# zer0int/OpenVision

Hardware: AMD Instinct MI355X
Metric: images/sec (node) ViT-L/14@224 fwd+InfoNCE (higher is better)
Workload: dtype bf16; 1 GPU; vit-large-patch14-224: image tower + text tower (T=80) + InfoNCE, per-GPU batch 256, formula weights, bf16 MFMA / fp32 accumulate; fp8_mask=0, global_batch=256, micro_batches=1, parallelism=dp1

## Files before the change

include/ovhip.h:

```cpp
#ifndef OVHIP_H
#define OVHIP_H

#include <stddef.h>
#include <stdint.h>

#ifdef __cplusplus
extern "C" {
#endif

#define OV_ABI_VERSION 2

typedef void* ov_stream_t;
typedef uint16_t ov_bf16;

enum ov_status {
    OV_OK = 0,
    OV_ERR_INVALID = -1,
    OV_ERR_UNSUPPORTED = -2,
    OV_ERR_WORKSPACE = -3,
    OV_ERR_NO_DEVICE = -4,
    OV_ERR_HIP = -1000
};

enum ov_dtype { OV_F32 = 0, OV_BF16 = 1 };
// ... 29 lines not shown
int ov_gemm_ln(const ov_bf16* X, int64_t ldx, const ov_bf16* Wg, int64_t ldw, const float* cvec, const float* colsum,
               const float* rowstats, ov_bf16* C, int64_t ldc, int64_t M, int N, int K, int epilogue, ov_stream_t stream);

int ov_gemm_keep(const ov_bf16* A, int64_t lda, const ov_bf16* W, int64_t ldw, const float* bias, ov_bf16* C, int64_t ldc,
                 ov_bf16* C2, int64_t ldc2, int64_t M, int N, int K, int epilogue, ov_stream_t stream);

int ov_rowstats(const ov_bf16* x, int64_t ldx, float* rowstats, int64_t rows, int D, float eps, ov_stream_t stream);

int ov_rowparts(const ov_bf16* x, int64_t ldx, float* parts, int64_t rows, int D, ov_stream_t stream);
int ov_rowstats_finalize(const float* parts, float* rowstats, int64_t rows, int D, float eps, ov_stream_t stream);
int ov_gemm_rowparts(const ov_bf16* A, int64_t lda, const ov_bf16* W, int64_t ldw, const float* bias, ov_bf16* C, int64_t ldc,
                     int64_t M, int N, int K, const ov_bf16* R, int64_t ldr, float* parts, ov_stream_t stream);

int ov_attention(const ov_bf16* qkv, int64_t ld_qkv, ov_bf16* out, int64_t ld_out,
                 int B, int L, int H, int hd, float scale, ov_stream_t stream);
int ov_attention_lse(const ov_bf16* qkv, int64_t ld_qkv, ov_bf16* out, int64_t ld_out, float* lse, int B, int L, int H, int hd, float scale,
                     ov_stream_t stream);
int ov_attention_prefix(const ov_bf16* qkv, int64_t ld_qkv, ov_bf16* out, int64_t ld_out, int B, int L, int H, int hd, float scale,
                        int prefix, ov_stream_t stream);

int ov_im2col_patches(const void* image, int img_dtype, ov_bf16* out, int B, int S, int P, int Kpad,
                      ov_stream_t stream);

int ov_im2col_patches_keep(const void* image, int img_dtype, const int* keep, ov_bf16* out, int B, int S, int P, int K, int Kpad,
                           ov_stream_t stream);
int ov_patch_keep_inverse(const int* keep, int* inv, int B, int K, int G, int* err_flag, ov_stream_t stream);
int ov_patch_keep_assemble(const ov_bf16* y, int64_t ldy, const float* cls, const float* pos, const int* keep, float* x, int B, int K,
                           int G, int D, ov_stream_t stream);
int ov_patch_keep_assemble_backward(const float* dx, const int* inv, int B, int K, int G, int D, float* dpos, float* dcls, ov_bf16* dy,
                                    int64_t lddy, ov_stream_t stream);
// ... 153 lines not shown
ov_tower* ov_tower_create(const ov_tower_cfg* cfg);
void      ov_tower_destroy(ov_tower* t);
int       ov_tower_set_block(ov_tower* t, int layer, const ov_block_weights* w);
int       ov_tower_set_block_fp8(ov_tower* t, int layer, const ov_block_fp8* q);
int       ov_tower_set_fp8_hidden_scale(ov_tower* t, float* amax, int mode);
#define OV_FP8_QKV 1
#define OV_FP8_OUT 2
#define OV_FP8_FC 4
#define OV_FP8_PROJ 8
#define OV_FP8_ALL 15
int       ov_tower_set_fp8_mask(ov_tower* t, const unsigned char* mask, int n);
int       ov_tower_set_prefix(ov_tower* t, int prefix);
size_t    ov_tower_workspace_bytes(const ov_tower* t, int B, int L);
int       ov_tower_forward(const ov_tower* t, ov_bf16* x, int B, int L, void* workspace,
                           size_t workspace_bytes, ov_stream_t stream);

typedef struct {
    float *ln1_w, *ln1_b;
    ov_bf16* qkv_w; float* qkv_b;
    ov_bf16* out_w; float* out_b;
    float *ln2_w, *ln2_b;
    ov_bf16* fc_w;  float* fc_b;
    ov_bf16* proj_w; float* proj_b;
} ov_block_grads;
typedef struct {
    const ov_bf16* qkv;
    const ov_bf16* attn_out;
    const ov_bf16* x1;
    const ov_bf16* fc_pre;
    const ov_bf16* ln1_out;
// ... 104 lines not shown
```

openvision_amd/_lib.py:

```python
from __future__ import annotations

import ctypes as C
import os
import threading

_PKG = os.path.dirname(os.path.abspath(__file__))
LIB_PATH = os.path.join(_PKG, "libovhip.so")
if os.environ.get("OVHIP_LIB"):
    LIB_PATH = os.path.join(_PKG, os.environ["OVHIP_LIB"]) if os.sep not in os.environ["OVHIP_LIB"] else os.environ["OVHIP_LIB"]

OV_F32, OV_BF16 = 0, 1
EPI_BIAS, EPI_GELU_ERF, EPI_GELU_TANH, EPI_RESIDUAL = 0, 1, 2, 3

c_void_p, c_int, c_int64, c_float, c_size_t = C.c_void_p, C.c_int, C.c_int64, C.c_float, C.c_size_t


class TowerCfg(C.Structure):
    _fields_ = [("width", c_int), ("layers", c_int), ("heads", c_int), ("mlp", c_int), ("mlp_pad", c_int),
                ("gelu_tanh", c_int), ("ln_eps", c_float)]


class BlockWeights(C.Structure):
    _fields_ = [(n, c_void_p) for n in ("ln1_w", "ln1_b", "qkv_w", "qkv_b", "out_w", "out_b", "ln2_w", "ln2_b",
                                        "fc_w", "fc_b", "proj_w", "proj_b", "qkv_colsum", "fc_colsum")]
# ... 42 lines not shown
                                   c_void_p, c_int64, c_int, c_int, c_int, c_void_p, c_int64, c_void_p]),
    "ov_tower_set_fp8_hidden_scale": (c_int, [c_void_p, c_void_p, c_int]),
    "ov_tower_set_fp8_mask": (c_int, [c_void_p, c_void_p, c_int]),
    "ov_layernorm_quant_fp8": (c_int, [c_void_p, c_int64, c_void_p, c_void_p, c_void_p, c_int64, c_void_p, c_int64, c_int, c_float,
                                       c_void_p]),
    "ov_gemm_ln": (c_int, [c_void_p, c_int64, c_void_p, c_int64, c_void_p, c_void_p, c_void_p, c_void_p, c_int64, c_int64, c_int,
                           c_int, c_int, c_void_p]),
    "ov_gemm_keep": (c_int, [c_void_p, c_int64, c_void_p, c_int64, c_void_p, c_void_p, c_int64, c_void_p, c_int64, c_int64, c_int, c_int,
                             c_int, c_void_p]),
    "ov_rowstats": (c_int, [c_void_p, c_int64, c_void_p, c_int64, c_int, c_float, c_void_p]),
    "ov_rowparts": (c_int, [c_void_p, c_int64, c_void_p, c_int64, c_int, c_void_p]),
    "ov_rowstats_finalize": (c_int, [c_void_p, c_void_p, c_int64, c_int, c_float, c_void_p]),
    "ov_gemm_rowparts": (c_int, [c_void_p, c_int64, c_void_p, c_int64, c_void_p, c_void_p, c_int64, c_int64, c_int, c_int, c_void_p, c_int64,
                                 c_void_p, c_void_p]),
    "ov_attention": (c_int, [c_void_p, c_int64, c_void_p, c_int64, c_int, c_int, c_int, c_int, c_float, c_void_p]),
    "ov_attention_prefix": (c_int, [c_void_p, c_int64, c_void_p, c_int64, c_int, c_int, c_int, c_int, c_float, c_int, c_void_p]),
    "ov_attention_prefix_backward_workspace_bytes": (c_size_t, [c_int, c_int, c_int, c_int]),
    "ov_attention_prefix_backward": (c_int, [c_void_p, c_int64, c_void_p, c_int64, c_void_p, c_int64, c_void_p, c_int64, c_int, c_int, c_int,
                                             c_int, c_float, c_int, c_void_p, c_size_t, c_void_p]),
    "ov_softmax_xent_workspace_bytes": (c_size_t, [c_int64]),
    "ov_softmax_xent": (c_int, [c_void_p, c_int64, c_void_p, c_void_p, c_int64, c_int, c_void_p, c_void_p, c_void_p, c_size_t, c_void_p]),
    "ov_softmax_xent_backward": (c_int, [c_void_p, c_int64, c_void_p, c_void_p, c_void_p, c_void_p, c_void_p, c_int64, c_int64, c_int,
                                         c_void_p, c_size_t, c_void_p]),
    "ov_tower_set_prefix": (c_int, [c_void_p, c_int]),
    "ov_block_backward_prefix": (c_int, [c_void_p, c_void_p, c_void_p, c_void_p, c_void_p, c_void_p, c_void_p, c_int, c_int, c_int, c_void_p,
                                         c_size_t, c_void_p]),
    "ov_im2col_patches": (c_int, [c_void_p, c_int, c_void_p, c_int, c_int, c_int, c_int, c_void_p]),
    "ov_im2col_patches_keep": (c_int, [c_void_p, c_int, c_void_p, c_void_p, c_int, c_int, c_int, c_int, c_int, c_void_p]),
    "ov_patch_keep_inverse": (c_int, [c_void_p, c_void_p, c_int, c_int, c_int, c_void_p, c_void_p]),
    "ov_patch_keep_assemble": (c_int, [c_void_p, c_int64, c_void_p, c_void_p, c_void_p, c_void_p, c_int, c_int, c_int, c_int, c_void_p]),
# ... 73 lines not shown
                                      c_void_p, c_void_p, c_void_p, c_void_p, c_void_p, c_void_p, c_void_p, c_size_t, c_void_p]),
    "ov_adamw_step": (c_int, [c_void_p, c_void_p, c_void_p, c_void_p, c_int64, c_float, c_float, c_float, c_float, c_float, c_int, c_float,
                              c_void_p, c_float, c_void_p]),
    "ov_sumsq_workspace_bytes": (c_size_t, []),
    "ov_sumsq": (c_int, [c_void_p, c_int64, c_void_p, c_int, c_void_p, c_size_t, c_void_p]),
    "ov_profile_enable": (c_int, [C.c_uint, c_int]),
    "ov_profile_read": (c_int, [c_int, C.POINTER(C.c_double), C.POINTER(c_int), C.POINTER(C.c_double)]),
    "ov_debug_gemm_stamps": (c_int, [c_void_p, c_int]),
    "ov_debug_gemm_wave_stamps": (c_int, [c_void_p]),
    "ov_tower_create": (c_void_p, [C.POINTER(TowerCfg)]),
    "ov_tower_destroy": (None, [c_void_p]),
    "ov_tower_set_block": (c_int, [c_void_p, c_int, C.POINTER(BlockWeights)]),
    "ov_tower_set_block_fp8": (c_int, [c_void_p, c_int, c_void_p]),
    "ov_tower_workspace_bytes": (c_size_t, [c_void_p, c_int, c_int]),
    "ov_tower_forward": (c_int, [c_void_p, c_void_p, c_int, c_int, c_void_p, c_size_t, c_void_p]),
    "ov_vision_workspace_bytes": (c_size_t, [c_void_p, C.POINTER(VisionHead), c_int]),
    "ov_vision_embed": (c_int, [c_void_p, C.POINTER(VisionHead), c_void_p, c_int, c_int, c_void_p, c_void_p, c_size_t,
                                c_void_p]),
    "ov_vision_head_forward": (c_int, [c_void_p, C.POINTER(VisionHead), c_void_p, c_int, c_void_p, c_int, c_void_p,
                                       c_size_t, c_void_p]),
    "ov_encode_image": (c_int, [c_void_p, C.POINTER(VisionHead), c_void_p, c_int, c_int, c_void_p, c_int, c_void_p,
                                c_size_t, c_void_p]),
    "ov_vision_head_forward_tokens": (c_int, [c_void_p, C.POINTER(VisionHead), c_void_p, c_int, c_int, c_void_p, c_int, c_void_p,
                                              c_size_t, c_void_p]),
    "ov_vision_keep_workspace_bytes": (c_size_t, [c_void_p, C.POINTER(VisionHead), c_int, c_int]),
    "ov_vision_embed_keep": (c_int, [c_void_p, C.POINTER(VisionHead), c_void_p, c_int, c_void_p, c_int, c_int, c_void_p, c_void_p,
                                     c_void_p, c_size_t, c_void_p]),
    "ov_encode_image_keep": (c_int, [c_void_p, C.POINTER(VisionHead), c_void_p, c_int, c_void_p, c_int, c_int, c_void_p, c_int,
                                     c_void_p, c_void_p, c_size_t, c_void_p]),
    "ov_text_workspace_bytes": (c_size_t, [c_void_p, C.POINTER(TextHead), c_int]),
# ... 48 lines not shown
```

openvision_amd/csrc/attention.hip:

```cpp
#include "common.h"
#include <stdlib.h>

namespace {

struct AttnArgs {
    const ov_bf16* qkv; int64_t ldq;
    ov_bf16* out; int64_t ldo;
    int B, L, H, nqt, KC;
    float scale_log2;
    int prefix;
};

typedef __attribute__((address_space(3))) s16x4_t* lds_s16x4_ptr;
typedef const __attribute__((address_space(1))) void* gptr_t;
typedef __attribute__((address_space(3))) void* lptr_t;

__device__ __forceinline__ bf16x8_t tr_pair(const char* p0, const char* p1) {
    const s16x4_t a = __builtin_amdgcn_ds_read_tr16_b64_v4i16((lds_s16x4_ptr)p0);
    const s16x4_t b = __builtin_amdgcn_ds_read_tr16_b64_v4i16((lds_s16x4_ptr)p1);
    typedef short s16x8_t __attribute__((ext_vector_type(8)));
    const s16x8_t c = {a[0], a[1], a[2], a[3], b[0], b[1], b[2], b[3]};
    return __builtin_bit_cast(bf16x8_t, c);
}

// ... 810 lines not shown
    const float inv = 1.0f / l;
    const int q = q0 + r;
    if (q < L) {
        ov_bf16* op = a.out + ((int64_t)b * L + q) * a.ldo + h * hd + 4 * h2;
#pragma unroll
        for (int t = 0; t < DT; ++t)
#pragma unroll
            for (int g = 0; g < 4; ++g) {
                const int d = t * 32 + 8 * g + 4 * h2;
                if (d < hd) {
                    const u32x2_t w = {pack_bf16x2(o[t][4 * g] * inv, o[t][4 * g + 1] * inv),
                                       pack_bf16x2(o[t][4 * g + 2] * inv, o[t][4 * g + 3] * inv)};
                    *(u32x2_t*)(op + t * 32 + 8 * g) = w;
                }
            }
    }
}

}

namespace {
int attention_impl(const ov_bf16* qkv, int64_t ld_qkv, ov_bf16* out, int64_t ld_out, int B, int L, int H, int hd, float scale,
                   const float* out_amax, float* amax_next, float* lse, ov_stream_t stream);
}

extern "C" int ov_attention(const ov_bf16* qkv, int64_t ld_qkv, ov_bf16* out, int64_t ld_out, int B, int L,
                            int H, int hd, float scale, ov_stream_t stream) {
    return attention_impl(qkv, ld_qkv, out, ld_out, B, L, H, hd, scale, nullptr, nullptr, nullptr, stream);
}

// ... 144 lines not shown
    static OvPerDeviceOnce attr;
    const int dev = ov_current_device();
    if (attr.need(dev)) {
        hipError_t e = hipFuncSetAttribute((const void*)attn_fwd_generic<64, true>, hipFuncAttributeMaxDynamicSharedMemorySize, 160 * 1024);
        if (e == hipSuccess)
            e = hipFuncSetAttribute((const void*)attn_fwd_generic<96, true>, hipFuncAttributeMaxDynamicSharedMemorySize, 160 * 1024);
        if (e != hipSuccess) return OV_ERR_HIP - (int)e;
        attr.mark(dev);
    }
    const dim3 grid((unsigned)(B * H), (unsigned)((g.nqt + nwg - 1) / nwg)), blk(nwg * 64);
    if (hdp == 64) hipLaunchKernelGGL((attn_fwd_generic<64, true>), grid, blk, smem, (hipStream_t)stream, g, hd);
    else hipLaunchKernelGGL((attn_fwd_generic<96, true>), grid, blk, smem, (hipStream_t)stream, g, hd);
    OV_LAUNCH_CHECK();
    return OV_OK;
}
```

openvision_amd/csrc/tower.hip:

```cpp
#include "common.h"
#include <new>
#include <vector>
#include <mutex>
#include <stdlib.h>

struct TailCtx {
    hipStream_t stream = nullptr;
    hipEvent_t fork = nullptr, join = nullptr;
    int state = 0;
    int device = -1;
    std::mutex mu;
};

struct ov_tower {
    mutable TailCtx tail;
    ov_tower_cfg cfg;
    ov_block_weights* blocks;
    unsigned char* set;
    ov_block_fp8* fp8;
    unsigned char* set8;
    float* h_amax;
    int h_mode;
    unsigned char* mask8;
    int prefix;
// ... 34 lines not shown
        e0 = g_prof.pool.back(); g_prof.pool.pop_back();
        e1 = g_prof.pool.back(); g_prof.pool.pop_back();
        on = true;
        (void)hipEventRecord(e0, st);
    }
    ~ProfScope() {
        if (!on) return;
        (void)hipEventRecord(e1, st);
        std::lock_guard<std::mutex> lk(g_prof.mu);
        g_prof.recs.push_back({cls, e0, e1, rows});
    }
};

inline size_t align_up(size_t x, size_t a) { return (x + a - 1) / a * a; }
inline int max_i(int a, int b) { return a > b ? a : b; }

struct VisionWs { size_t x, tower, pooled, lnrow, feat, total; };
inline VisionWs vision_ws(const ov_tower* t, const ov_vision_head* h, int B) {
    const int g = h->image_size / h->patch_size, L = g * g + 1, D = t->cfg.width;
    VisionWs w;
    size_t off = 0;
    w.x = off;      off += align_up((size_t)B * L * D * 2, 256);
    w.tower = off;  off += align_up(ov_tower_workspace_bytes(t, B, L), 256);
    w.pooled = off; off += align_up((size_t)B * D * 4, 256);
    w.lnrow = off;  off += align_up((size_t)B * D * 2, 256);
    w.feat = off;   off += align_up((size_t)B * h->embed_pad * 2, 256);
    w.total = off;
    return w;
}
inline size_t keep_embed_bytes(const ov_tower* t, const ov_vision_head* h, int B, int K) {
// ... 187 lines not shown
    }
    return OV_OK;
}

extern "C" int ov_tower_set_prefix(ov_tower* t, int prefix) {
    if (!t || prefix < -1) return OV_ERR_INVALID;
    t->prefix = prefix;
    return OV_OK;
}

extern "C" size_t ov_tower_workspace_bytes(const ov_tower* t, int B, int L) {
    if (!t || B <= 0 || L <= 0) return 0;
    const size_t M = (size_t)B * L;
    const int D = t->cfg.width;
    size_t n = align_up(M * D * 2, 256) + align_up(M * (size_t)big_pitch(t->cfg) * 2, 256) + align_up(M * 8, 256) +
               align_up(M * (size_t)(D / 32) * 8, 256);
    if (tower_fp8(t)) n += align_up(M * (size_t)max_i(D, t->cfg.mlp_pad), 256) + align_up(M * 4, 256);
    return n;
}

namespace {
struct BlockPart { ov_bf16 *x, *h, *big; float *stats, *parts; unsigned char* q8; float* qs; int B; ov_stream_t stream; bool prof; };
struct Fp8Scales { float *h_amax, *a_amax, *h_next, *a_next; int h_mode; };

int run_block(const ov_tower_cfg& c, const ov_block_weights& w, const ov_block_fp8* q, int mask, const Fp8Scales& sc, const BlockPart& p,
              bool parts_in, int L, int prefix) {
    const int D = c.width, H = c.heads, hd = D / H, F = c.mlp_pad, B = p.B;
    const int64_t M = (int64_t)B * L;
    const int ldb = big_pitch(c);
    const float scale = 1.0f / sqrtf((float)hd);
// ... 59 lines not shown
        else if (fold) OV_STEP(fc_cls, ov_gemm_ln(x, D, w.fc_w, D, w.fc_b, w.fc_colsum, stats, big, ldb, M, F, D, gelu, stream));
        else OV_STEP(fc_cls, ov_gemm(h, D, w.fc_w, D, w.fc_b, big, ldb, M, F, D, gelu, nullptr, 0, 0, 0, 0, stream));
        if (f_proj) {
            OV_STEP(OV_PROF_LN, ov_quant_rows_fp8(big, ldb, q8, F, qs, M, F, (sc.h_mode == 1 && f_fc) ? sc.h_amax : nullptr, stream));
            OV_STEP(OV_PROF_GEMM_PROJ, ov_gemm_fp8(q8, F, q->proj_w8, F, qs, q->proj_s, w.proj_b, x, D, M, D, F, OV_EPI_BIAS_RESIDUAL, x, D, stream));
        } else if (rp) {
            OV_STEP(OV_PROF_GEMM_PROJ, ov_gemm_rowparts(big, ldb, w.proj_w, F, w.proj_b, x, D, M, D, F, x, D, parts, stream));
        } else {
            OV_STEP(OV_PROF_GEMM_PROJ, ov_gemm(big, ldb, w.proj_w, F, w.proj_b, x, D, M, D, F, OV_EPI_BIAS_RESIDUAL, x, D, 0, 0, 0, stream));
        }
    }
#undef OV_STEP
    return OV_OK;
}

TailCtx* tail_ctx(const ov_tower* t) {
    TailCtx& tc = t->tail;
    std::lock_guard<std::mutex> lk(tc.mu);
    if (tc.state == 0) {
        const char* e = getenv("OVHIP_NO_TAIL_SPLIT");
        if (e && e[0] == '1') { tc.state = -1; return nullptr; }
        tc.device = ov_current_device();
        if (hipStreamCreateWithFlags(&tc.stream, hipStreamNonBlocking) == hipSuccess &&
            hipEventCreateWithFlags(&tc.fork, hipEventDisableTiming) == hipSuccess &&
            hipEventCreateWithFlags(&tc.join, hipEventDisableTiming) == hipSuccess)
            tc.state = 1;
        else
            tc.state = -1;
    }
    return tc.state == 1 && tc.device == ov_current_device() ? &tc : nullptr;
}

int tail_images(int B, int L) {
    const int64_t T = ((int64_t)B * L + 255) / 256;
    const int r = (int)(T % 64);
    if (T <= 64 || r == 0 || r > 8) return 0;
    const int64_t target = T - r;
    int Bm = (int)((target * 256) / L);
    while (Bm > 0 && ((int64_t)Bm * L + 255) / 256 > target) --Bm;
    const int tail = B - Bm;
    if (Bm <= 0 || tail <= 0 || tail > B / 8) return 0;
    return tail;
}
}

extern "C" int ov_tower_forward(const ov_tower* t, ov_bf16* x, int B, int L, void* workspace, size_t workspace_bytes,
                                ov_stream_t stream) {
    if (!t || !x || !workspace || B <= 0 || L <= 0) return OV_ERR_INVALID;
    if (workspace_bytes < ov_tower_workspace_bytes(t, B, L)) return OV_ERR_WORKSPACE;
    if (((uintptr_t)x | (uintptr_t)workspace) & 15) return OV_ERR_INVALID;
    const ov_tower_cfg& c = t->cfg;
    const int D = c.width;
    const int64_t M = (int64_t)B * L;
    const int ldb = big_pitch(c);
    ov_bf16* h = (ov_bf16*)workspace;
    ov_bf16* big = (ov_bf16*)((char*)workspace + align_up((size_t)M * D * 2, 256));
    float* stats = (float*)((char*)big + align_up((size_t)M * ldb * 2, 256));
    for (int i = 0; i < c.layers; ++i)
        if (!t->set[i]) return OV_ERR_INVALID;

    int nt = tail_images(B, L);
    TailCtx* tc = nt > 0 ? tail_ctx(t) : nullptr;
    if (!tc) nt = 0;
    const int Bm = B - nt;
    hipStream_t main_st = (hipStream_t)stream;
// ... 7 lines not shown
    const int64_t off = (int64_t)Bm * L;
    const bool fp8 = tower_fp8(t);
    if (t->prefix >= 0 && fp8) return OV_ERR_UNSUPPORTED;
    if (t->prefix > L) return OV_ERR_INVALID;
    int rc = OV_OK;
    if (fp8 && t->h_amax && t->h_mode == 2)
        rc = ov_amax_roll(t->h_amax, t->h_amax + 2 * c.layers, 2 * c.layers, stream);
    const int G = D / 32;
    float* parts = use_rowparts() && !fp8 ? (float*)((char*)workspace + ov_tower_workspace_bytes(t, B, L) - align_up((size_t)M * G * 8, 256)) : nullptr;
    const int qw = D > c.mlp_pad ? D : c.mlp_pad;
    unsigned char* q8 = (unsigned char*)stats + align_up((size_t)M * 8, 256);
    float* qs = (float*)(q8 + align_up((size_t)M * qw, 256));
    const BlockPart main_part = {x, h, big, stats, parts, q8, qs, Bm, stream, true};
    const BlockPart tail_part = {x + off * D, h + off * D, big + off * ldb, stats + 2 * off, parts ? parts + 2 * off * G : nullptr,
                                 q8 + off * qw, qs + off, nt, (ov_stream_t)(nt > 0 ? tc->stream : nullptr), false};
    for (int i = 0; i < c.layers && rc == OV_OK; ++i) {
        Fp8Scales sc = {nullptr, nullptr, nullptr, nullptr, 0};
        if (t->h_amax) sc = {t->h_amax + i, t->h_amax + c.layers + i, t->h_amax + 2 * c.layers + i, t->h_amax + 3 * c.layers + i, t->h_mode};
        const ov_block_fp8* q = fp8 ? &t->fp8[i] : nullptr;
        const int mask = fp8 ? t->mask8[i] : 0;
        rc = run_block(c, t->blocks[i], q, mask, sc, main_part, i > 0, L, t->prefix);
        if (rc == OV_OK && nt > 0) rc = run_block(c, t->blocks[i], q, mask, sc, tail_part, i > 0, L, t->prefix);
    }
    if (nt > 0) {
        hipError_t e = hipEventRecord(tc->join, tc->stream);
        if (e == hipSuccess) e = hipStreamWaitEvent(main_st, tc->join, 0);
        if (e != hipSuccess && rc == OV_OK) rc = OV_ERR_HIP - (int)e;
    }
    return rc;
}

int block_grad_pairs(const ov_block_grads* g);
int block_backward_partial(const ov_tower_cfg* cfg, const ov_block_weights* w, const ov_bf16* x, const ov_block_saved* s, const ov_bf16* dy,
                           ov_bf16* dx, const ov_block_grads* g, int prefix, int B, int L, void* workspace, size_t workspace_bytes,
                           ov_stream_t stream);
size_t block_backward_input_workspace_bytes(const ov_tower_cfg* cfg, int B, int L);
int block_backward_input(const ov_tower_cfg* cfg, const ov_block_weights* w, const ov_bf16* x, const ov_block_saved* s, const ov_bf16* dy,
                         ov_bf16* dx, int prefix, int B, int L, void* workspace, ov_stream_t stream);

static inline size_t saved_per_token(const ov_tower_cfg& c) { return (size_t)8 * c.width + 2 * (size_t)c.mlp_pad; }
static inline size_t saved_lse_elems(const ov_tower_cfg& c, int B, int L) {
    return ((size_t)2 * B * c.heads * ((L + 31) / 32 * 32) + 7) / 8 * 8;
}
static inline size_t saved_per_layer(const ov_tower_cfg& c, int B, int L) { return (size_t)B * L * saved_per_token(c) + saved_lse_elems(c, B, L); }
// ... 255 lines not shown
    int rc;
    if ((rc = ov_im2col_patches(image, img_dtype, patches, B, h->image_size, h->patch_size, h->kpad, stream))) return rc;
    if ((rc = ov_gemm(patches, h->kpad, h->conv_w, h->kpad, nullptr, x, D, (int64_t)B * g * g, D, h->kpad,
                      OV_EPI_BIAS_RESIDUAL, h->pos, D, g * g, g * g, 1, stream)))
        return rc;
    return ov_cls_rows(x, D, h->cls, h->pos_f32, B, L, D, stream);
}

extern "C" int ov_vision_head_forward(const ov_tower* t, const ov_vision_head* h, const ov_bf16* x, int B, float* features,
                                      int normalize, void* workspace, size_t workspace_bytes, ov_stream_t stream) {
    if (!t || !h || !x || !features || !workspace || B <= 0 || h->patch_size <= 0) return OV_ERR_INVALID;
    const int g = h->image_size / h->patch_size;
    return ov_vision_head_forward_tokens(t, h, x, B, g * g + 1, features, normalize, workspace, workspace_bytes, stream);
}

extern "C" int ov_vision_head_forward_tokens(const ov_tower* t, const ov_vision_head* h, const ov_bf16* x, int B, int L, float* features,
                                             int normalize, void* workspace, size_t workspace_bytes, ov_stream_t stream) {
    if (!t || !h || !x || !features || !workspace || B <= 0 || L < 2) return OV_ERR_INVALID;
    const int D = t->cfg.width, E = h->embed_dim, EP = h->embed_pad;
    if (EP % 8 || EP < E) return OV_ERR_INVALID;
    if (!h->final_ln_after_pool) return OV_ERR_UNSUPPORTED;
    const size_t o_pooled = 0, o_ln = align_up((size_t)B * D * 4, 256), o_feat = o_ln + align_up((size_t)B * D * 2, 256);
    if (workspace_bytes < o_feat + (size_t)B * EP * 2) return OV_ERR_WORKSPACE;
    float* pooled = (float*)((char*)workspace + o_pooled);
    ov_bf16* ln = (ov_bf16*)((char*)workspace + o_ln);
    ov_bf16* feat = (ov_bf16*)((char*)workspace + o_feat);
    int rc;
    if (h->pool_avg) {
        if ((rc = ov_mean_pool(x, D, pooled, B, L, D, 1, stream))) return rc;
        if ((rc = ov_layernorm(pooled, OV_F32, D, h->ln_post_w, h->ln_post_b, ln, OV_BF16, D, B, D, t->cfg.ln_eps, stream))) return rc;
    } else {
        if ((rc = ov_layernorm(x, OV_BF16, (int64_t)L * D, h->ln_post_w, h->ln_post_b, ln, OV_BF16, D, B, D, t->cfg.ln_eps, stream)))
            return rc;
    }
    if ((rc = ov_gemm(ln, D, h->proj_t, D, nullptr, feat, EP, B, EP, D, OV_EPI_BIAS, nullptr, 0, 0, 0, 0, stream))) return rc;
    if (normalize) return ov_l2norm(feat, OV_BF16, EP, features, E, B, E, stream);
    return ov_convert(feat, OV_BF16, EP, features, OV_F32, E, B, E, stream);
}

extern "C" int ov_encode_image(const ov_tower* t, const ov_vision_head* h, const void* image, int img_dtype, int B,
                               float* features, int normalize, void* workspace, size_t workspace_bytes, ov_stream_t stream) {
    if (!t || !h || !image || !features || !workspace || B <= 0) return OV_ERR_INVALID;
    const VisionWs w = vision_ws(t, h, B);
    if (workspace_bytes < w.total) return OV_ERR_WORKSPACE;
    const int g = h->image_size / h->patch_size, L = g * g + 1;
    char* ws = (char*)workspace;
    ov_bf16* x = (ov_bf16*)(ws + w.x);
    const size_t tower_bytes = ov_tower_workspace_bytes(t, B, L);
    int rc;
    if ((size_t)B * g * g * h->kpad * 2 > tower_bytes) return OV_ERR_WORKSPACE;
    if ((rc = ov_vision_embed(t, h, image, img_dtype, B, x, ws + w.tower, tower_bytes, stream))) return rc;
    if ((rc = ov_tower_forward(t, x, B, L, ws + w.tower, tower_bytes, stream))) return rc;
    return ov_vision_head_forward(t, h, x, B, features, normalize, ws + w.pooled, w.total - w.pooled, stream);
}

int ov_im2col_patches_keep_pos(const void* image, int img_dtype, const int* keep, ov_bf16* out, int B, int S, int P, int K, int Kpad,
                               const ov_bf16* pos, ov_bf16* posk, int D, int* err_flag, ov_stream_t stream);

extern "C" size_t ov_vision_keep_workspace_bytes(const ov_tower* t, const ov_vision_head* h, int B, int K) {
    if (!t || !h || B <= 0 || h->patch_size <= 0) return 0;
    const int g = h->image_size / h->patch_size;
    if (K < 1 || K > g * g) return 0;
    return vision_keep_ws(t, h, B, K).total;
}

extern "C" int ov_vision_embed_keep(const ov_tower* t, const ov_vision_head* h, const void* image, int img_dtype, const int* keep, int B,
                                    int K, ov_bf16* x, int* err_flag, void* workspace, size_t workspace_bytes, ov_stream_t stream) {
    if (!t || !h || !image || !keep || !x || !workspace || B <= 0 || h->patch_size <= 0) return OV_ERR_INVALID;
// ... 14 lines not shown
}

extern "C" int ov_encode_image_keep(const ov_tower* t, const ov_vision_head* h, const void* image, int img_dtype, const int* keep, int B,
                                    int K, float* features, int normalize, int* err_flag, void* workspace, size_t workspace_bytes,
                                    ov_stream_t stream) {
    if (!t || !h || !image || !keep || !features || !workspace || B <= 0 || h->patch_size <= 0) return OV_ERR_INVALID;
    const int g = h->image_size / h->patch_size;
    if (K < 1 || K > g * g) return OV_ERR_INVALID;
    const VisionWs w = vision_keep_ws(t, h, B, K);
    if (workspace_bytes < w.total) return OV_ERR_WORKSPACE;
    const int L = K + 1;
    char* ws = (char*)workspace;
    ov_bf16* x = (ov_bf16*)(ws + w.x);
    int rc;
    if ((rc = ov_vision_embed_keep(t, h, image, img_dtype, keep, B, K, x, err_flag, ws + w.tower, w.pooled - w.tower, stream))) return rc;
    if ((rc = ov_tower_forward(t, x, B, L, ws + w.tower, w.pooled - w.tower, stream))) return rc;
    return ov_vision_head_forward_tokens(t, h, x, B, L, features, normalize, ws + w.pooled, w.total - w.pooled, stream);
}

extern "C" size_t ov_text_workspace_bytes(const ov_tower* t, const ov_text_head* h, int B) {
    if (!t || !h || B <= 0) return 0;
    return text_ws(t, h, B).total;
}

extern "C" int ov_encode_text(const ov_tower* t, const ov_text_head* h, const int64_t* tokens, int B, float* features,
                              int normalize, int* err_flag, void* workspace, size_t workspace_bytes, ov_stream_t stream) {
    if (!t || !h || !tokens || !features || !workspace || B <= 0) return OV_ERR_INVALID;
    const TextWs w = text_ws(t, h, B);
    if (workspace_bytes < w.total) return OV_ERR_WORKSPACE;
    const int T = h->context_length, D = t->cfg.width, E = h->embed_dim, EP = (E + 7) / 8 * 8;
    char* ws = (char*)workspace;
    ov_bf16* x = (ov_bf16*)(ws + w.x);
    ov_bf16* last = (ov_bf16*)(ws + w.last);
    ov_bf16* ln = (ov_bf16*)(ws + w.lnrow);
    ov_bf16* feat = (ov_bf16*)(ws + w.feat);
    int rc;
    if ((rc = ov_text_embed(tokens, h->token_embedding, h->pos, x, D, B, T, D, h->vocab_size, err_flag, stream))) return rc;
    if ((rc = ov_tower_forward(t, x, B, T, ws + w.tower, ov_tower_workspace_bytes(t, B, T), stream))) return rc;
    if ((rc = ov_gather_rows(x, D, last, D, B, T, h->pool_last ? T - 1 : 0, D, stream))) return rc;
    if ((rc = ov_layernorm(last, OV_BF16, D, h->ln_final_w, h->ln_final_b, ln, OV_BF16, D, B, D, t->cfg.ln_eps, stream))) return rc;
    if ((rc = ov_gemm(ln, D, h->proj_t, D, nullptr, feat, EP, B, EP, D, OV_EPI_BIAS, nullptr, 0, 0, 0, 0, stream))) return rc;
    if (normalize) return ov_l2norm(feat, OV_BF16, EP, features, E, B, E, stream);
    return ov_convert(feat, OV_BF16, EP, features, OV_F32, E, B, E, stream);
}
```

Before: 5690 images/sec.

## Compute only pooled token rows in final transformer block

The last transformer block now computes K/V for all tokens but runs Q projection, attention, output projection, LN2 and the MLP only for the pooled row (CLS for vision, last/first token for text). A new row-wise attention kernel handles single query rows against full K/V. This removes most of the final layer's GEMM and attention cost in both towers. It adds a separate code path with extra workspace and a scalar attention kernel, and falls back to the full path for fp8 or prefix modes.

Result: no change. 5716 images/sec, median of 6 (+0.5%).

```diff
diff --git a/include/ovhip.h b/include/ovhip.h
--- a/include/ovhip.h
+++ b/include/ovhip.h
@@ -67,6 +67,8 @@
 
 int ov_attention(const ov_bf16* qkv, int64_t ld_qkv, ov_bf16* out, int64_t ld_out,
                  int B, int L, int H, int hd, float scale, ov_stream_t stream);
+int ov_attention_rows(const ov_bf16* q, int64_t ldq, const ov_bf16* kv, int64_t ldkv, ov_bf16* out, int64_t ldo,
+                      int B, int L, int H, int hd, float scale, ov_stream_t stream);
 int ov_attention_lse(const ov_bf16* qkv, int64_t ld_qkv, ov_bf16* out, int64_t ld_out, float* lse, int B, int L, int H, int hd, float scale,
                      ov_stream_t stream);
 int ov_attention_prefix(const ov_bf16* qkv, int64_t ld_qkv, ov_bf16* out, int64_t ld_out, int B, int L, int H, int hd, float scale,
@@ -250,6 +252,8 @@
 size_t    ov_tower_workspace_bytes(const ov_tower* t, int B, int L);
 int       ov_tower_forward(const ov_tower* t, ov_bf16* x, int B, int L, void* workspace,
                            size_t workspace_bytes, ov_stream_t stream);
+int       ov_tower_forward_pooled(const ov_tower* t, ov_bf16* x, int B, int L, int row, ov_bf16* out_rows, void* workspace,
+                                  size_t workspace_bytes, ov_stream_t stream);
 
 typedef struct {
     float *ln1_w, *ln1_b;
diff --git a/openvision_amd/_lib.py b/openvision_amd/_lib.py
--- a/openvision_amd/_lib.py
+++ b/openvision_amd/_lib.py
@@ -80,6 +80,7 @@
     "ov_gemm_rowparts": (c_int, [c_void_p, c_int64, c_void_p, c_int64, c_void_p, c_void_p, c_int64, c_int64, c_int, c_int, c_void_p, c_int64,
                                  c_void_p, c_void_p]),
     "ov_attention": (c_int, [c_void_p, c_int64, c_void_p, c_int64, c_int, c_int, c_int, c_int, c_float, c_void_p]),
+    "ov_attention_rows": (c_int, [c_void_p, c_int64, c_void_p, c_int64, c_void_p, c_int64, c_int, c_int, c_int, c_int, c_float, c_void_p]),
     "ov_attention_prefix": (c_int, [c_void_p, c_int64, c_void_p, c_int64, c_int, c_int, c_int, c_int, c_float, c_int, c_void_p]),
     "ov_attention_prefix_backward_workspace_bytes": (c_size_t, [c_int, c_int, c_int, c_int]),
     "ov_attention_prefix_backward": (c_int, [c_void_p, c_int64, c_void_p, c_int64, c_void_p, c_int64, c_void_p, c_int64, c_int, c_int, c_int,
@@ -183,6 +184,7 @@
     "ov_tower_set_block_fp8": (c_int, [c_void_p, c_int, c_void_p]),
     "ov_tower_workspace_bytes": (c_size_t, [c_void_p, c_int, c_int]),
     "ov_tower_forward": (c_int, [c_void_p, c_void_p, c_int, c_int, c_void_p, c_size_t, c_void_p]),
+    "ov_tower_forward_pooled": (c_int, [c_void_p, c_void_p, c_int, c_int, c_int, c_void_p, c_void_p, c_size_t, c_void_p]),
     "ov_vision_workspace_bytes": (c_size_t, [c_void_p, C.POINTER(VisionHead), c_int]),
     "ov_vision_embed": (c_int, [c_void_p, C.POINTER(VisionHead), c_void_p, c_int, c_int, c_void_p, c_void_p, c_size_t,
                                 c_void_p]),
diff --git a/openvision_amd/csrc/attention.hip b/openvision_amd/csrc/attention.hip
--- a/openvision_amd/csrc/attention.hip
+++ b/openvision_amd/csrc/attention.hip
@@ -848,6 +848,107 @@
                     *(u32x2_t*)(op + t * 32 + 8 * g) = w;
                 }
             }
+    }
+}
+
+struct AttnRowArgs {
+    const ov_bf16* q; int64_t ldq;
+    const ov_bf16* kv; int64_t ldkv;
+    ov_bf16* out; int64_t ldo;
+    int L, H, hd;
+    float scale_log2;
+};
+constexpr int ROW_KEYS = 128;
+constexpr int ROW_NCHP = 13;
+
+__device__ __forceinline__ void unpack8(u32x4_t w, float (&f)[8]) {
+#pragma unroll
+    for (int e = 0; e < 4; ++e) { f[2 * e] = bf16lo_to_f32(w[e]); f[2 * e + 1] = bf16hi_to_f32(w[e]); }
+}
+
+__global__ __launch_bounds__(64) void attn_fwd_rows(const AttnRowArgs a) {
+    __shared__ float part[ROW_KEYS * ROW_NCHP];
+    __shared__ float sp[ROW_KEYS];
+    __shared__ float so[64 * 8];
+    const int lane = threadIdx.x;
+    const int bh = blockIdx.x, b = bh / a.H, h = bh - b * a.H;
+    const int L = a.L, hd = a.hd, nch = hd >> 3, nchp = nch | 1, HD = a.H * hd;
+    const int kpi = 64 / nch;
+    const int vk = lane / nch, vc = lane - vk * nch;
+    const bool act = vk < kpi;
+    const ov_bf16* kb = a.kv + (int64_t)b * L * a.ldkv + h * hd + (act ? vc : 0) * 8;
+    const ov_bf16* vb = kb + HD;
+    float qf[8], o[8];
+    unpack8(*(const u32x4_t*)(a.q + (int64_t)b * a.ldq + h * hd + (act ? vc : 0) * 8), qf);
+#pragma unroll
+    for (int e = 0; e < 8; ++e) o[e] = 0.f;
+    float m = -INFINITY, l = 0.f;
+    for (int c0 = 0; c0 < L; c0 += ROW_KEYS) {
+        const int nk = L - c0 < ROW_KEYS ? L - c0 : ROW_KEYS;
+        if (act) {
+#pragma unroll 4
+            for (int j = vk; j < nk; j += kpi) {
+                float kf[8];
+                unpack8(*(const u32x4_t*)(kb + (int64_t)(c0 + j) * a.ldkv), kf);
+                float d = 0.f;
+#pragma unroll
+                for (int e = 0; e < 8; ++e) d = fmaf(kf[e], qf[e], d);
+                part[j * nchp + vc] = d;
+            }
+        }
+        __syncthreads();
+        float s[2] = {0.f, 0.f};
+#pragma unroll
+        for (int i = 0; i < 2; ++i)
+            if (lane + 64 * i < nk)
+                for (int c = 0; c < nch; ++c) s[i] += part[(lane + 64 * i) * nchp + c];
+        float mx = -INFINITY;
+#pragma unroll
+        for (int i = 0; i < 2; ++i)
+            if (lane + 64 * i < nk) mx = fmaxf(mx, s[i] * a.scale_log2);
+        mx = wave_max(mx);
+        const float mn = fmaxf(m, mx);
+        const float alpha = __builtin_amdgcn_exp2f(m - mn);
+        float ps = 0.f;
+#pragma unroll
+        for (int i = 0; i < 2; ++i) {
+            if (lane + 64 * i < nk) {
+                const float p = __builtin_amdgcn_exp2f(fmaf(s[i], a.scale_log2, -mn));
+                sp[lane + 64 * i] = p;
+                ps += p;
+            }
+        }
+        l = fmaf(l, alpha, wave_sum(ps));
+        m = mn;
+#pragma unroll
+        for (int e = 0; e < 8; ++e) o[e] *= alpha;
+        __syncthreads();
+        if (act) {
+#pragma unroll 4
+            for (int j = vk; j < nk; j += kpi) {
+                float vf[8];
+                unpack8(*(const u32x4_t*)(vb + (int64_t)(c0 + j) * a.ldkv), vf);
+                const float p = sp[j];
+#pragma unroll
+                for (int e = 0; e < 8; ++e) o[e] = fmaf(p, vf[e], o[e]);
+            }
+        }
+        __syncthreads();
+    }
+#pragma unroll
+    for (int e = 0; e < 8; ++e) so[lane * 8 + e] = o[e];
+    __syncthreads();
+    if (lane < nch) {
+        const float inv = 1.0f / l;
+        float r[8];
+#pragma unroll
+        for (int e = 0; e < 8; ++e) r[e] = 0.f;
+        for (int k = 0; k < kpi; ++k)
+#pragma unroll
+            for (int e = 0; e < 8; ++e) r[e] += so[(k * nch + lane) * 8 + e];
+        const u32x4_t w = {pack_bf16x2(r[0] * inv, r[1] * inv), pack_bf16x2(r[2] * inv, r[3] * inv),
+                           pack_bf16x2(r[4] * inv, r[5] * inv), pack_bf16x2(r[6] * inv, r[7] * inv)};
+        *(u32x4_t*)(a.out + (int64_t)b * a.ldo + h * hd + lane * 8) = w;
     }
 }
 
@@ -1022,3 +1123,19 @@
     OV_LAUNCH_CHECK();
     return OV_OK;
 }
+
+extern "C" int ov_attention_rows(const ov_bf16* q, int64_t ldq, const ov_bf16* kv, int64_t ldkv, ov_bf16* out, int64_t ldo, int B, int L,
+                                 int H, int hd, float scale, ov_stream_t stream) {
+    if (!q || !kv || !out || B <= 0 || L <= 0 || H <= 0) return OV_ERR_INVALID;
+    if (hd <= 0 || hd % 8 || hd > 96) return OV_ERR_UNSUPPORTED;
+    if (ldq % 8 || ldkv % 8 || ldo % 8 || ldq < H * hd || ldkv < 2 * H * hd || ldo < H * hd) return OV_ERR_INVALID;
+    if (((uintptr_t)q | (uintptr_t)kv | (uintptr_t)out) & 15) return OV_ERR_INVALID;
+    if ((int64_t)B * H > 0x7fffffffLL) return OV_ERR_UNSUPPORTED;
+    AttnRowArgs r;
+    r.q = q; r.ldq = ldq; r.kv = kv; r.ldkv = ldkv; r.out = out; r.ldo = ldo;
+    r.L = L; r.H = H; r.hd = hd;
+    r.scale_log2 = scale * 1.4426950408889634f;
+    hipLaunchKernelGGL(attn_fwd_rows, dim3((unsigned)(B * H)), dim3(64), 0, (hipStream_t)stream, r);
+    OV_LAUNCH_CHECK();
+    return OV_OK;
+}
diff --git a/openvision_amd/csrc/tower.hip b/openvision_amd/csrc/tower.hip
--- a/openvision_amd/csrc/tower.hip
+++ b/openvision_amd/csrc/tower.hip
@@ -72,6 +72,20 @@
 
 inline size_t align_up(size_t x, size_t a) { return (x + a - 1) / a * a; }
 inline int max_i(int a, int b) { return a > b ? a : b; }
+
+struct PooledWs { ov_bf16 *xr, *n, *q, *o, *hid; float* stats; };
+inline size_t pooled_ws_bytes(const ov_tower_cfg& c, int B) {
+    return 4 * align_up((size_t)B * c.width * 2, 256) + align_up((size_t)B * c.mlp_pad * 2, 256) + align_up((size_t)B * 8, 256);
+}
+inline PooledWs pooled_ws(const ov_tower_cfg& c, void* base, int B) {
+    const size_t row = align_up((size_t)B * c.width * 2, 256);
+    char* p = (char*)base;
+    PooledWs w;
+    w.xr = (ov_bf16*)p; w.n = (ov_bf16*)(p + row); w.q = (ov_bf16*)(p + 2 * row); w.o = (ov_bf16*)(p + 3 * row);
+    w.hid = (ov_bf16*)(p + 4 * row);
+    w.stats = (float*)(p + 4 * row + align_up((size_t)B * c.mlp_pad * 2, 256));
+    return w;
+}
 
 struct VisionWs { size_t x, tower, pooled, lnrow, feat, total; };
 inline VisionWs vision_ws(const ov_tower* t, const ov_vision_head* h, int B) {
@@ -289,6 +303,7 @@
     const size_t M = (size_t)B * L;
     const int D = t->cfg.width;
     size_t n = align_up(M * D * 2, 256) + align_up(M * (size_t)big_pitch(t->cfg) * 2, 256) + align_up(M * 8, 256) +
+               pooled_ws_bytes(t->cfg, B) +
                align_up(M * (size_t)(D / 32) * 8, 256);
     if (tower_fp8(t)) n += align_up(M * (size_t)max_i(D, t->cfg.mlp_pad), 256) + align_up(M * 4, 256);
     return n;
@@ -378,6 +393,52 @@
     return OV_OK;
 }
 
+int run_block_pooled(const ov_tower_cfg& c, const ov_block_weights& w, const BlockPart& p, int L, int row, const PooledWs& pw, ov_bf16* out) {
+    const int D = c.width, H = c.heads, hd = D / H, F = c.mlp_pad, B = p.B;
+    const int64_t M = (int64_t)B * L;
+    const int ldb = big_pitch(c);
+    const float scale = 1.0f / sqrtf((float)hd);
+    const int gelu = c.gelu_tanh ? OV_EPI_BIAS_GELU_TANH : OV_EPI_BIAS_GELU_ERF;
+    const int fc_cls = c.gelu_tanh ? OV_PROF_GEMM_FC_TANH : OV_PROF_GEMM_FC;
+    const bool fold = w.qkv_colsum != nullptr && w.fc_colsum != nullptr;
+    const ov_bf16* x = p.x;
+    ov_bf16* kv = p.big + D;
+    ov_stream_t stream = p.stream;
+    int rc;
+#define OV_STEP(cls, rows, call)                                         \
+    do {                                                                 \
+        if (p.prof) { ProfScope ps__(cls, stream, rows); rc = (call); }  \
+        else rc = (call);                                                \
+        if (rc) return rc;                                               \
+    } while (0)
+    if ((rc = ov_gather_rows(x, D, pw.xr, D, B, L, row, D, stream))) return rc;
+    if (fold) {
+        OV_STEP(OV_PROF_LN, M, ov_rowstats(x, D, p.stats, M, D, c.ln_eps, stream));
+        OV_STEP(OV_PROF_GEMM_QKV, M, ov_gemm_ln(x, D, w.qkv_w + (size_t)D * D, D, w.qkv_b + D, w.qkv_colsum + D, p.stats, kv, ldb, M, 2 * D, D,
+                                                OV_EPI_BIAS, stream));
+        OV_STEP(OV_PROF_LN, B, ov_rowstats(pw.xr, D, pw.stats, B, D, c.ln_eps, stream));
+        OV_STEP(OV_PROF_GEMM_QKV, B, ov_gemm_ln(pw.xr, D, w.qkv_w, D, w.qkv_b, w.qkv_colsum, pw.stats, pw.q, D, B, D, D, OV_EPI_BIAS, stream));
+    } else {
+        OV_STEP(OV_PROF_LN, M, ov_layernorm(x, OV_BF16, D, w.ln1_w, w.ln1_b, p.h, OV_BF16, D, M, D, c.ln_eps, stream));
+        OV_STEP(OV_PROF_GEMM_QKV, M, ov_gemm(p.h, D, w.qkv_w + (size_t)D * D, D, w.qkv_b + D, kv, ldb, M, 2 * D, D, OV_EPI_BIAS, nullptr, 0, 0, 0, 0,
+                                             stream));
+        if ((rc = ov_gather_rows(p.h, D, pw.n, D, B, L, row, D, stream))) return rc;
+        OV_STEP(OV_PROF_GEMM_QKV, B, ov_gemm(pw.n, D, w.qkv_w, D, w.qkv_b, pw.q, D, B, D, D, OV_EPI_BIAS, nullptr, 0, 0, 0, 0, stream));
+    }
+    OV_STEP(OV_PROF_ATTN, B, ov_attention_rows(pw.q, D, kv, ldb, pw.o, D, B, L, H, hd, scale, stream));
+    OV_STEP(OV_PROF_GEMM_OUT, B, ov_gemm(pw.o, D, w.out_w, D, w.out_b, pw.xr, D, B, D, D, OV_EPI_BIAS_RESIDUAL, pw.xr, D, 0, 0, 0, stream));
+    if (fold) {
+        OV_STEP(OV_PROF_LN, B, ov_rowstats(pw.xr, D, pw.stats, B, D, c.ln_eps, stream));
+        OV_STEP(fc_cls, B, ov_gemm_ln(pw.xr, D, w.fc_w, D, w.fc_b, w.fc_colsum, pw.stats, pw.hid, F, B, F, D, gelu, stream));
+    } else {
+        OV_STEP(OV_PROF_LN, B, ov_layernorm(pw.xr, OV_BF16, D, w.ln2_w, w.ln2_b, pw.n, OV_BF16, D, B, D, c.ln_eps, stream));
+        OV_STEP(fc_cls, B, ov_gemm(pw.n, D, w.fc_w, D, w.fc_b, pw.hid, F, B, F, D, gelu, nullptr, 0, 0, 0, 0, stream));
+    }
+    OV_STEP(OV_PROF_GEMM_PROJ, B, ov_gemm(pw.hid, F, w.proj_w, F, w.proj_b, out, D, B, D, F, OV_EPI_BIAS_RESIDUAL, pw.xr, D, 0, 0, 0, stream));
+#undef OV_STEP
+    return OV_OK;
+}
+
 TailCtx* tail_ctx(const ov_tower* t) {
     TailCtx& tc = t->tail;
     std::lock_guard<std::mutex> lk(tc.mu);
@@ -408,11 +469,8 @@
 }
 }
 
-extern "C" int ov_tower_forward(const ov_tower* t, ov_bf16* x, int B, int L, void* workspace, size_t workspace_bytes,
-                                ov_stream_t stream) {
-    if (!t || !x || !workspace || B <= 0 || L <= 0) return OV_ERR_INVALID;
-    if (workspace_bytes < ov_tower_workspace_bytes(t, B, L)) return OV_ERR_WORKSPACE;
-    if (((uintptr_t)x | (uintptr_t)workspace) & 15) return OV_ERR_INVALID;
+static int tower_walk(const ov_tower* t, ov_bf16* x, int B, int L, void* workspace, ov_stream_t stream, int nblocks, int row,
+                      ov_bf16* out_rows) {
     const ov_tower_cfg& c = t->cfg;
     const int D = c.width;
     const int64_t M = (int64_t)B * L;
@@ -450,7 +508,7 @@
     const BlockPart main_part = {x, h, big, stats, parts, q8, qs, Bm, stream, true};
     const BlockPart tail_part = {x + off * D, h + off * D, big + off * ldb, stats + 2 * off, parts ? parts + 2 * off * G : nullptr,
                                  q8 + off * qw, qs + off, nt, (ov_stream_t)(nt > 0 ? tc->stream : nullptr), false};
-    for (int i = 0; i < c.layers && rc == OV_OK; ++i) {
+    for (int i = 0; i < nblocks && rc == OV_OK; ++i) {
         Fp8Scales sc = {nullptr, nullptr, nullptr, nullptr, 0};
         if (t->h_amax) sc = {t->h_amax + i, t->h_amax + c.layers + i, t->h_amax + 2 * c.layers + i, t->h_amax + 3 * c.layers + i, t->h_mode};
         const ov_block_fp8* q = fp8 ? &t->fp8[i] : nullptr;
@@ -463,7 +521,31 @@
         if (e == hipSuccess) e = hipStreamWaitEvent(main_st, tc->join, 0);
         if (e != hipSuccess && rc == OV_OK) rc = OV_ERR_HIP - (int)e;
     }
+    if (rc == OV_OK && nblocks < c.layers) {
+        const BlockPart all = {x, h, big, stats, nullptr, nullptr, nullptr, B, stream, true};
+        rc = run_block_pooled(c, t->blocks[nblocks], all, L, row, pooled_ws(c, (char*)stats + align_up((size_t)M * 8, 256), B), out_rows);
+    }
     return rc;
+}
+
+extern "C" int ov_tower_forward(const ov_tower* t, ov_bf16* x, int B, int L, void* workspace, size_t workspace_bytes,
+                                ov_stream_t stream) {
+    if (!t || !x || !workspace || B <= 0 || L <= 0) return OV_ERR_INVALID;
+    if (workspace_bytes < ov_tower_workspace_bytes(t, B, L)) return OV_ERR_WORKSPACE;
+    if (((uintptr_t)x | (uintptr_t)workspace) & 15) return OV_ERR_INVALID;
+    return tower_walk(t, x, B, L, workspace, stream, t->cfg.layers, 0, nullptr);
+}
+
+extern "C" int ov_tower_forward_pooled(const ov_tower* t, ov_bf16* x, int B, int L, int row, ov_bf16* out_rows, void* workspace,
+                                       size_t workspace_bytes, ov_stream_t stream) {
+    if (!t || !x || !out_rows || !workspace || B <= 0 || L <= 0 || row < 0 || row >= L) return OV_ERR_INVALID;
+    if (workspace_bytes < ov_tower_workspace_bytes(t, B, L)) return OV_ERR_WORKSPACE;
+    if (((uintptr_t)x | (uintptr_t)out_rows | (uintptr_t)workspace) & 15) return OV_ERR_INVALID;
+    if (tower_fp8(t) || t->prefix >= 0) {
+        const int rc = tower_walk(t, x, B, L, workspace, stream, t->cfg.layers, 0, nullptr);
+        return rc ? rc : ov_gather_rows(x, t->cfg.width, out_rows, t->cfg.width, B, L, row, t->cfg.width, stream);
+    }
+    return tower_walk(t, x, B, L, workspace, stream, t->cfg.layers - 1, row, out_rows);
 }
 
 int block_grad_pairs(const ov_block_grads* g);
@@ -749,9 +831,8 @@
     return ov_vision_head_forward_tokens(t, h, x, B, g * g + 1, features, normalize, workspace, workspace_bytes, stream);
 }
 
-extern "C" int ov_vision_head_forward_tokens(const ov_tower* t, const ov_vision_head* h, const ov_bf16* x, int B, int L, float* features,
-                                             int normalize, void* workspace, size_t workspace_bytes, ov_stream_t stream) {
-    if (!t || !h || !x || !features || !workspace || B <= 0 || L < 2) return OV_ERR_INVALID;
+static int vision_head(const ov_tower* t, const ov_vision_head* h, const ov_bf16* x, int B, int L, int64_t tok_pitch, float* features,
+                       int normalize, void* workspace, size_t workspace_bytes, ov_stream_t stream) {
     const int D = t->cfg.width, E = h->embed_dim, EP = h->embed_pad;
     if (EP % 8 || EP < E) return OV_ERR_INVALID;
     if (!h->final_ln_after_pool) return OV_ERR_UNSUPPORTED;
@@ -765,12 +846,33 @@
         if ((rc = ov_mean_pool(x, D, pooled, B, L, D, 1, stream))) return rc;
         if ((rc = ov_layernorm(pooled, OV_F32, D, h->ln_post_w, h->ln_post_b, ln, OV_BF16, D, B, D, t->cfg.ln_eps, stream))) return rc;
     } else {
-        if ((rc = ov_layernorm(x, OV_BF16, (int64_t)L * D, h->ln_post_w, h->ln_post_b, ln, OV_BF16, D, B, D, t->cfg.ln_eps, stream)))
+        if ((rc = ov_layernorm(x, OV_BF16, tok_pitch > 0 ? tok_pitch : (int64_t)L * D, h->ln_post_w, h->ln_post_b, ln, OV_BF16, D, B, D,
+                               t->cfg.ln_eps, stream)))
             return rc;
     }
     if ((rc = ov_gemm(ln, D, h->proj_t, D, nullptr, feat, EP, B, EP, D, OV_EPI_BIAS, nullptr, 0, 0, 0, 0, stream))) return rc;
     if (normalize) return ov_l2norm(feat, OV_BF16, EP, features, E, B, E, stream);
     return ov_convert(feat, OV_BF16, EP, features, OV_F32, E, B, E, stream);
+}
+
+extern "C" int ov_vision_head_forward_tokens(const ov_tower* t, const ov_vision_head* h, const ov_bf16* x, int B, int L, float* features,
+                                             int normalize, void* workspace, size_t workspace_bytes, ov_stream_t stream) {
+    if (!t || !h || !x || !features || !workspace || B <= 0 || L < 2) return OV_ERR_INVALID;
+    return vision_head(t, h, x, B, L, 0, features, normalize, workspace, workspace_bytes, stream);
+}
+
+static int vision_blocks_head(const ov_tower* t, const ov_vision_head* h, ov_bf16* x, int B, int L, float* features, int normalize,
+                              void* tower_ws, size_t tower_bytes, void* head_ws, size_t head_bytes, ov_stream_t stream) {
+    int rc;
+    if (h->pool_avg) {
+        if ((rc = ov_tower_forward(t, x, B, L, tower_ws, tower_bytes, stream))) return rc;
+        return ov_vision_head_forward_tokens(t, h, x, B, L, features, normalize, head_ws, head_bytes, stream);
+    }
+    if (!h->final_ln_after_pool) return OV_ERR_UNSUPPORTED;
+    if (head_bytes < (size_t)B * t->cfg.width * 2) return OV_ERR_WORKSPACE;
+    ov_bf16* cls_rows = (ov_bf16*)head_ws;
+    if ((rc = ov_tower_forward_pooled(t, x, B, L, 0, cls_rows, tower_ws, tower_bytes, stream))) return rc;
+    return vision_head(t, h, cls_rows, B, L, t->cfg.width, features, normalize, head_ws, head_bytes, stream);
 }
 
 extern "C" int ov_encode_image(const ov_tower* t, const ov_vision_head* h, const void* image, int img_dtype, int B,
@@ -785,8 +887,7 @@
     int rc;
     if ((size_t)B * g * g * h->kpad * 2 > tower_bytes) return OV_ERR_WORKSPACE;
     if ((rc = ov_vision_embed(t, h, image, img_dtype, B, x, ws + w.tower, tower_bytes, stream))) return rc;
-    if ((rc = ov_tower_forward(t, x, B, L, ws + w.tower, tower_bytes, stream))) return rc;
-    return ov_vision_head_forward(t, h, x, B, features, normalize, ws + w.pooled, w.total - w.pooled, stream);
+    return vision_blocks_head(t, h, x, B, L, features, normalize, ws + w.tower, tower_bytes, ws + w.pooled, w.total - w.pooled, stream);
 }
 
 int ov_im2col_patches_keep_pos(const void* image, int img_dtype, const int* keep, ov_bf16* out, int B, int S, int P, int K, int Kpad,
@@ -831,8 +932,7 @@
     ov_bf16* x = (ov_bf16*)(ws + w.x);
     int rc;
     if ((rc = ov_vision_embed_keep(t, h, image, img_dtype, keep, B, K, x, err_flag, ws + w.tower, w.pooled - w.tower, stream))) return rc;
-    if ((rc = ov_tower_forward(t, x, B, L, ws + w.tower, w.pooled - w.tower, stream))) return rc;
-    return ov_vision_head_forward_tokens(t, h, x, B, L, features, normalize, ws + w.pooled, w.total - w.pooled, stream);
+    return vision_blocks_head(t, h, x, B, L, features, normalize, ws + w.tower, w.pooled - w.tower, ws + w.pooled, w.total - w.pooled, stream);
 }
 
 extern "C" size_t ov_text_workspace_bytes(const ov_tower* t, const ov_text_head* h, int B) {
@@ -853,8 +953,8 @@
     ov_bf16* feat = (ov_bf16*)(ws + w.feat);
     int rc;
     if ((rc = ov_text_embed(tokens, h->token_embedding, h->pos, x, D, B, T, D, h->vocab_size, err_flag, stream))) return rc;
-    if ((rc = ov_tower_forward(t, x, B, T, ws + w.tower, ov_tower_workspace_bytes(t, B, T), stream))) return rc;
-    if ((rc = ov_gather_rows(x, D, last, D, B, T, h->pool_last ? T - 1 : 0, D, stream))) return rc;
+    if ((rc = ov_tower_forward_pooled(t, x, B, T, h->pool_last ? T - 1 : 0, last, ws + w.tower, ov_tower_workspace_bytes(t, B, T), stream)))
+        return rc;
     if ((rc = ov_layernorm(last, OV_BF16, D, h->ln_final_w, h->ln_final_b, ln, OV_BF16, D, B, D, t->cfg.ln_eps, stream))) return rc;
     if ((rc = ov_gemm(ln, D, h->proj_t, D, nullptr, feat, EP, B, EP, D, OV_EPI_BIAS, nullptr, 0, 0, 0, 0, stream))) return rc;
     if (normalize) return ov_l2norm(feat, OV_BF16, EP, features, E, B, E, stream);
```
